# sohamazing/image-stitcher

Measured on AMD Instinct MI355X. Metric: stitched Mvoxels/s, higher is better.
Workload: dtype u16

## Files before the change

### image-stitcher_amd/csrc/fuse.hip

```cpp
#include <hip/hip_runtime.h>

#include <algorithm>
#include <cstdlib>
#include <map>

#include "common.h"

using namespace sq;

namespace {

typedef uint32_t u32x4 __attribute__((ext_vector_type(4)));
typedef float f32x4 __attribute__((ext_vector_type(4)));
typedef double f64x2 __attribute__((ext_vector_type(2)));

struct __attribute__((packed)) U32x4U {
    u32x4 v;
};
struct __attribute__((packed)) F32x4U {
    f32x4 v;
};
typedef uint32_t u32x2 __attribute__((ext_vector_type(2)));
struct __attribute__((packed)) U32x2U {
    u32x2 v;
// ... 1697 lines not shown
        }
    }
}

template <typename K>
int launch(K kernel, const FuseParams &P, int64_t n_items, int n_planes, hipStream_t stream, int grid_override = 0) {
    const int64_t n_work = n_items * n_planes;
    if (n_work == 0) return SQ_OK;
    static thread_local std::map<const void *, int> resident;
    const void *key = reinterpret_cast<const void *>(kernel);
    auto it = resident.find(key);
    if (it == resident.end()) {
        int dev = 0, cus = 256, per_cu = 8;
        hipDeviceProp_t prop;
        if (hipGetDevice(&dev) == hipSuccess && hipGetDeviceProperties(&prop, dev) == hipSuccess)
            cus = prop.multiProcessorCount;
        if (hipOccupancyMaxActiveBlocksPerMultiprocessor(&per_cu, kernel, 256, 0) != hipSuccess || per_cu < 1) per_cu = 4;
        it = resident.emplace(key, cus * std::min(per_cu, 8)).first;
    }
    const int64_t blocks = std::min<int64_t>(n_work, grid_override > 0 ? grid_override : it->second);
    FuseParams Q = P;
    Q.chunk = (int32_t)std::max<int64_t>(1, std::min<int64_t>(QUEUE_CHUNK, n_work / (blocks * 16)));
    hipLaunchKernelGGL(kernel, dim3((unsigned)blocks), dim3(256), 0, stream, Q, n_items, n_work);
    hipError_t e = hipGetLastError();
    if (e != hipSuccess) return fail(SQ_ERR_HIP, "sq_fuse_planes: launch failed: %s", hipGetErrorString(e));
    return SQ_OK;
}

template <typename K>
int launch_zg(K kernel, const FuseParams &P, int64_t n_items, int n_planes, hipStream_t stream, int grid_override) {
    if (n_items == 0 || n_planes == 0) return SQ_OK;
    static thread_local std::map<const void *, int> resident;
    const void *key = reinterpret_cast<const void *>(kernel);
    auto it = resident.find(key);
    if (it == resident.end()) {
        int dev = 0, cus = 256, per_cu = 8;
        hipDeviceProp_t prop;
        if (hipGetDevice(&dev) == hipSuccess && hipGetDeviceProperties(&prop, dev) == hipSuccess)
            cus = prop.multiProcessorCount;
        if (hipOccupancyMaxActiveBlocksPerMultiprocessor(&per_cu, kernel, 256, 0) != hipSuccess || per_cu < 1) per_cu = 4;
        it = resident.emplace(key, cus * std::min(per_cu, 8)).first;
    }
    const int64_t min_units = n_items * ((n_planes + ZB - 1) / ZB);
    const int64_t blocks = std::min<int64_t>(min_units, grid_override > 0 ? grid_override : it->second);
    FuseParams Q = P;
    Q.chunk = (int32_t)std::max<int64_t>(1, std::min<int64_t>(QUEUE_CHUNK, min_units / (blocks * 16)));
    hipLaunchKernelGGL(kernel, dim3((unsigned)blocks), dim3(256), 0, stream, Q, n_items);
    hipError_t e = hipGetLastError();
    if (e != hipSuccess) return fail(SQ_ERR_HIP, "sq_fuse_planes: launch failed: %s", hipGetErrorString(e));
    return SQ_OK;
}

template <typename G>
__global__ __launch_bounds__(256) void flat_classify_kernel(const void *const *flat_ptrs, int64_t n, uint32_t *cls) {
    const int plane = blockIdx.y;
    const G *f = static_cast<const G *>(flat_ptrs[plane]);
    if (!f) return;
    for (int q = 0; q < plane; ++q)
        if (flat_ptrs[q] == f) return;
    const G lo = (G)__builtin_ldexp(1.0, FAST_MIN_EXP), hi = (G)__builtin_ldexp(1.0, FAST_END_EXP);
    const G mlo = (G)__builtin_ldexp(1.0, -MODERATE_EXP), mhi = (G)__builtin_ldexp(1.0, MODERATE_EXP);
    bool odd = false, wide = false, neg = false;
    auto look = [&](G g) {
        const G a = g < 0 ? -g : g;
        odd |= !(a >= lo && a < hi);
        wide |= !(a >= mlo && a < mhi);
        neg |= !(g > 0);
    };
    constexpr int PER = 16 / sizeof(G);
    const int64_t head = min<int64_t>(n, (int64_t)((16 - (reinterpret_cast<uintptr_t>(f) & 15)) & 15) / (int64_t)sizeof(G));
    const int64_t nvec = (n - head) / PER;
    const int64_t tid = (int64_t)blockIdx.x * blockDim.x + threadIdx.x, nthr = (int64_t)gridDim.x * blockDim.x;
    for (int64_t v = tid; v < nvec; v += nthr) {
        if constexpr (sizeof(G) == 4) {
            const f32x4 q = *reinterpret_cast<const f32x4 *>(f + head + v * PER);
            look(q[0]), look(q[1]), look(q[2]), look(q[3]);
        } else {
            const F64x2U q = *reinterpret_cast<const F64x2U *>(f + head + v * PER);
            look(q.v[0]), look(q.v[1]);
        }
    }
    for (int64_t i = tid; i < head; i += nthr) look(ldg_s<G>(f + i));
    for (int64_t i = head + nvec * PER + tid; i < n; i += nthr) look(ldg_s<G>(f + i));
    const uint32_t bits = (__builtin_amdgcn_ballot_w64(odd) ? 1u : 0u) | (__builtin_amdgcn_ballot_w64(wide) ? 2u : 0u) |
                          (__builtin_amdgcn_ballot_w64(neg) ? 4u : 0u);
    if (bits && (threadIdx.x & 63) == 0) atomicOr(&cls[plane], bits);
}

__global__ __launch_bounds__(256) void flat_class_share_kernel(const void *const *flat_ptrs, int n_planes, uint32_t *cls) {
    for (int p = threadIdx.x; p < n_planes; p += 256) {
        const void *f = flat_ptrs[p];
        if (!f) continue;
        for (int q = 0; q < p; ++q)
            if (flat_ptrs[q] == f) {
                cls[p] = cls[q];
                break;
            }
    }
}

__global__ __launch_bounds__(256) void selftest_divide_kernel(int exponent0, int negative, unsigned long long *bad) {
    const uint32_t mant = blockIdx.x * 256u + threadIdx.x;
    const int exponent = exponent0 + (int)blockIdx.y;
    const uint32_t bits = ((uint32_t)(exponent + 127) << 23) | mant | (negative ? 0x80000000u : 0u);
    const float g = __uint_as_float(bits);
    unsigned long long local = 0;
    for (int v = 0; v < 65536; ++v)
    {
        const uint32_t want = flat_f32<uint16_t>((uint16_t)v, g);
        const uint32_t pair = flat_f32_fast_pair((uint32_t)v | ((uint32_t)v << 16), g, g);
        local += want != flat_f32_fast<uint16_t>((uint16_t)v, g);
        local += want != (pair & 0xFFFFu);
        local += want != (pair >> 16);
        local += flat_f32<uint16_t, 1>((uint16_t)v, g) != flat_f32_fast<uint16_t, 1>((uint16_t)v, g);
        local += __fdiv_rn((float)v, g) != div_u16_normal_ieee((float)v, g);
    }
    for (int off = 32; off > 0; off >>= 1) local += __shfl_xor(local, off);
    if ((threadIdx.x & 63) == 0 && local) atomicAdd(bad, local);
}

}

extern "C" int sq_selftest_flat_divide(int32_t exponent, int32_t n_binades, int32_t negative, uint64_t *mismatches_dev,
                                       void *stream) {
    if (!mismatches_dev || exponent < FAST_MIN_EXP || n_binades < 1 || exponent + n_binades > FAST_END_EXP)
        return fail(SQ_ERR_INVALID, "sq_selftest_flat_divide: binades [%d, %d] outside the fast path's range [%d, %d]",
                    exponent, exponent + n_binades - 1, FAST_MIN_EXP, FAST_END_EXP - 1);
    hipStream_t s = static_cast<hipStream_t>(stream);
    hipError_t e = hipMemsetAsync(mismatches_dev, 0, sizeof(uint64_t), s);
    if (e == hipSuccess) {
        hipLaunchKernelGGL(selftest_divide_kernel, dim3(1u << 15, n_binades), dim3(256), 0, s, exponent, negative,
                           reinterpret_cast<unsigned long long *>(mismatches_dev));
        e = hipGetLastError();
    }
    if (e != hipSuccess) return fail(SQ_ERR_HIP, "sq_selftest_flat_divide: %s", hipGetErrorString(e));
    return SQ_OK;
}

__global__ __launch_bounds__(256) void selftest_blend_divide_kernel(int exponent0, int negative, unsigned long long *bad) {
    const uint32_t mant = blockIdx.x * 256u + threadIdx.x;
    const int exponent = exponent0 + (int)blockIdx.y;
    const float acc = __uint_as_float(((uint32_t)(exponent + 127) << 23) | mant | (negative ? 0x80000000u : 0u));
    unsigned long long local = 0;
    for (int ws = 2; ws <= BLEND_WSUM_MAX; ++ws) {
        const float d = (float)ws;
        const float want = __fdiv_rn(acc, d), got = div_by_refined(acc, d, recip_for<1>(d));
        local += __float_as_uint(want) != __float_as_uint(got);
    }
    if (local) atomicAdd(bad, local);
}

// ... 42 lines not shown
    if (!mismatches_dev || exponent < FAST_MIN_EXP || n_binades < 1 || exponent + n_binades > FAST_END_EXP)
        return fail(SQ_ERR_INVALID, "sq_selftest_flat_divide_f64: binades [%d, %d] outside the fast path's range [%d, %d]",
                    exponent, exponent + n_binades - 1, FAST_MIN_EXP, FAST_END_EXP - 1);
    hipStream_t s = static_cast<hipStream_t>(stream);
    hipError_t e = hipMemsetAsync(mismatches_dev, 0, sizeof(uint64_t), s);
    if (e == hipSuccess) {
        hipLaunchKernelGGL(selftest_divide_f64_kernel, dim3(128, n_binades), dim3(256), 0, s, exponent, negative, seed,
                           reinterpret_cast<unsigned long long *>(mismatches_dev));
        e = hipGetLastError();
    }
    if (e != hipSuccess) return fail(SQ_ERR_HIP, "sq_selftest_flat_divide_f64: %s", hipGetErrorString(e));
    return SQ_OK;
}

namespace {
struct ScratchLayout {
    int64_t queue, n_groups, groups, total;
};
ScratchLayout scratch_layout(int64_t n_planes) {
    ScratchLayout L;
    L.queue = (n_planes * 4 + 127) & ~int64_t(127);
    L.n_groups = L.queue + 9 * QUEUE_STRIDE * 4;
    L.groups = L.n_groups + 128;
    L.total = L.groups + n_planes * (int64_t)sizeof(PlaneGroup);
    return L;
}
}

extern "C" int64_t sq_fuse_scratch_bytes(int32_t n_planes) {
    if (n_planes < 0) return fail(SQ_ERR_INVALID, "sq_fuse_scratch_bytes: n_planes %d", n_planes);
    return scratch_layout(n_planes).total;
}

extern "C" int sq_fuse_planes(const sq_fuse_args *a, void *stream_) {
    if (!a || !a->plan || !a->table_dev || !a->canvas_dev)
        return fail(SQ_ERR_INVALID, "sq_fuse_planes: NULL plan/table/canvas");
    const TableHeader &h = a->plan->header();
    if (a->plan->spans_only && !a->plan->expanded)
        return fail(SQ_ERR_INVALID, "sq_fuse_planes: the plan of sq_fuse_plan_create_spans has not been through sq_fuse_plan_expand");
    if (a->table_bytes != a->plan->device_bytes())
        return fail(SQ_ERR_INVALID, "sq_fuse_planes: table_bytes %lld != plan %lld", (long long)a->table_bytes,
                    (long long)a->plan->device_bytes());
    if (a->mode != h.mode) return fail(SQ_ERR_INVALID, "sq_fuse_planes: mode %d but plan was built for %d", a->mode, h.mode);
    if (a->n_tiles != h.n_tiles || a->tile_h != h.tile_h || a->tile_w != h.tile_w || a->canvas_h != h.canvas_h ||
        a->canvas_w != h.canvas_w)
        return fail(SQ_ERR_INVALID, "sq_fuse_planes: geometry differs from the plan (tiles %d/%d %dx%d/%dx%d canvas %dx%d/%dx%d)",
                    a->n_tiles, h.n_tiles, a->tile_h, a->tile_w, h.tile_h, h.tile_w, a->canvas_h, a->canvas_w, h.canvas_h,
                    h.canvas_w);
    if (!a->tile_ptrs_dev && !a->tile_base_dev && h.n_refs > 0)
        return fail(SQ_ERR_INVALID, "sq_fuse_planes: no tile table and no tile base");
    if (a->tile_pitch < a->tile_w || a->canvas_pitch < a->canvas_w)
        return fail(SQ_ERR_INVALID, "sq_fuse_planes: pitch smaller than width");
    if (a->n_planes < 0) return fail(SQ_ERR_INVALID, "sq_fuse_planes: n_planes %d out of range", a->n_planes);
    if ((a->flags & ~(SQ_FUSE_FORCE_QUEUES | SQ_FUSE_FORCE_STATIC | SQ_FUSE_NO_PLANE_GROUPS | SQ_FUSE_NO_SEAM_OWNERS | SQ_FUSE_CONSECUTIVE_GROUPS)) || a->grid_blocks < 0 ||
        ((a->flags & SQ_FUSE_FORCE_QUEUES) && (a->flags & SQ_FUSE_FORCE_STATIC)))
        return fail(SQ_ERR_INVALID, "sq_fuse_planes: flags %d / grid_blocks %d", a->flags, a->grid_blocks);
    if (a->tile_dtype != SQ_U8 && a->tile_dtype != SQ_U16)
        return fail(SQ_ERR_UNSUPPORTED, "sq_fuse_planes: tile dtype %d (uint8/uint16 only)", a->tile_dtype);
    if (a->flat_ptrs_dev && a->flat_dtype != SQ_F32 && a->flat_dtype != SQ_F64)
        return fail(SQ_ERR_UNSUPPORTED, "sq_fuse_planes: flatfield dtype %d (float32/float64 only)", a->flat_dtype);
    if (a->canvas_plane_stride < (int64_t)a->canvas_h * a->canvas_pitch && a->n_planes > 1)
        return fail(SQ_ERR_INVALID, "sq_fuse_planes: canvas planes overlap");
    const size_t esz = a->canvas_dtype == SQ_F32 ? 4 : (size_t)a->canvas_dtype;
    if (reinterpret_cast<uintptr_t>(a->canvas_dev) % esz)
        return fail(SQ_ERR_INVALID, "sq_fuse_planes: canvas pointer not aligned to its element size");

    FuseParams P{};
    const char *base = static_cast<const char *>(a->table_dev);
    P.spans = reinterpret_cast<const Span *>(base + h.off_spans);
    P.refs = reinterpret_cast<const Ref *>(base + h.off_refs);
    P.items = reinterpret_cast<const Item *>(base + h.off_items);
    P.seams = (h.off_seams && !(a->flags & SQ_FUSE_NO_SEAM_OWNERS)) ? reinterpret_cast<const Seam *>(base + h.off_seams) : nullptr;
    P.tile_ptrs = a->tile_ptrs_dev;
    P.tile_base = a->tile_base_dev;
    P.tile_plane_stride = a->tile_plane_stride;
    P.tile_stride = a->tile_stride;
    P.flat_ptrs = a->flat_ptrs_dev;
    P.canvas = a->canvas_dev;
    P.canvas_plane_stride = a->canvas_plane_stride;
    P.n_tiles = a->n_tiles;
    P.tile_h = a->tile_h;
    P.tile_w = a->tile_w;
    P.tile_pitch = a->tile_pitch;
    P.canvas_pitch = a->canvas_pitch;
    P.flat_class = nullptr;
    hipStream_t stream = static_cast<hipStream_t>(stream_);
    const int flat = a->flat_ptrs_dev ? (a->flat_dtype == SQ_F64 ? 2 : 1) : 0;
    P.queue = nullptr;
    P.lane_items = (int32_t)h.lane_items;
    P.n_planes = a->n_planes;
    const ScratchLayout SL = scratch_layout(a->n_planes);
    if (a->scratch_dev && a->n_planes > 0) {
        if (a->scratch_bytes < sq_fuse_scratch_bytes(a->n_planes))
            return fail(SQ_ERR_WORKSPACE, "sq_fuse_planes: scratch %lld < %lld bytes", (long long)a->scratch_bytes,
                        (long long)sq_fuse_scratch_bytes(a->n_planes));
        if (reinterpret_cast<uintptr_t>(a->scratch_dev) % 128) return fail(SQ_ERR_INVALID, "sq_fuse_planes: scratch not 128-byte aligned");
        if (hipMemsetAsync(a->scratch_dev, 0, (size_t)SL.groups, stream) != hipSuccess)
            return fail(SQ_ERR_HIP, "sq_fuse_planes: cannot clear the scratch");
        if (flat) {
            if (flat == 1)
                hipLaunchKernelGGL(flat_classify_kernel<float>, dim3(256, a->n_planes), dim3(256), 0, stream, a->flat_ptrs_dev,
                                   (int64_t)a->tile_h * a->tile_w, static_cast<uint32_t *>(a->scratch_dev));
            else
                hipLaunchKernelGGL(flat_classify_kernel<double>, dim3(256, a->n_planes), dim3(256), 0, stream, a->flat_ptrs_dev,
                                   (int64_t)a->tile_h * a->tile_w, static_cast<uint32_t *>(a->scratch_dev));
            if (a->n_planes > 1)
                hipLaunchKernelGGL(flat_class_share_kernel, dim3(1), dim3(256), 0, stream, a->flat_ptrs_dev, a->n_planes,
                                   static_cast<uint32_t *>(a->scratch_dev));
            P.flat_class = static_cast<const uint32_t *>(a->scratch_dev);
        }
        const int64_t n_work = (int64_t)a->n_planes * h.n_items;
        if ((n_work >= 100000 || (a->flags & SQ_FUSE_FORCE_QUEUES)) && n_work < (int64_t(1) << 31) && !(a->flags & SQ_FUSE_FORCE_STATIC))
            P.queue = reinterpret_cast<uint32_t *>(static_cast<char *>(a->scratch_dev) + SL.queue);
    }
    const bool u16 = a->tile_dtype == SQ_U16;
    const bool grouping = a->scratch_dev && a->n_planes > 1 && ZB > 1 && !(a->flags & SQ_FUSE_NO_PLANE_GROUPS);
    auto build_groups = [&](const void *const *gains, uint32_t cls_mask) {
        char *sc = static_cast<char *>(a->scratch_dev);
        uint32_t *n_groups = reinterpret_cast<uint32_t *>(sc + SL.n_groups);
        PlaneGroup *groups = reinterpret_cast<PlaneGroup *>(sc + SL.groups);
        hipLaunchKernelGGL(build_groups_kernel, dim3(1), dim3(256), 0, stream, gains, P.flat_class, cls_mask, a->n_planes,
                           a->canvas_plane_stride * (int64_t)esz, ZB, n_groups, groups,
                           (a->flags & SQ_FUSE_CONSECUTIVE_GROUPS) != 0);
        P.groups = groups;
        P.n_groups = n_groups;
    };

    if (a->mode == SQ_FUSE_OVERWRITE) {
        if (a->canvas_dtype != a->tile_dtype)
            return fail(SQ_ERR_INVALID, "sq_fuse_planes: overwrite mode keeps the tile dtype (canvas %d, tile %d)",
                        a->canvas_dtype, a->tile_dtype);
#define SQ_OVERWRITE(T, F)                                                                                  \
    do {                                                                                                      \
        if (P.queue) return launch(fuse_overwrite_kernel<T, F, true>, P, h.n_items, a->n_planes, stream, a->grid_blocks);     \
        return launch(fuse_overwrite_kernel<T, F, false>, P, h.n_items, a->n_planes, stream, a->grid_blocks);                 \
    } while (0)
        if (flat && grouping) {
            build_groups(a->flat_ptrs_dev, 1u);
#define SQ_ZG(G, T)                                                                                                                  \
    do {                                                                                                                              \
        if (P.queue) return launch_zg(fuse_overwrite_zg_kernel<G, true, T>, P, h.n_items, a->n_planes, stream, a->grid_blocks);       \
        return launch_zg(fuse_overwrite_zg_kernel<G, false, T>, P, h.n_items, a->n_planes, stream, a->grid_blocks);                   \
    } while (0)
            if (u16) {
                if (flat == 2) SQ_ZG(double, uint16_t);
                SQ_ZG(float, uint16_t);
            }
            if (flat == 2) SQ_ZG(double, uint8_t);
            SQ_ZG(float, uint8_t);
        }
        if (u16 && !flat && grouping) {
            build_groups(nullptr, 0u);
            SQ_ZG(NoGain, uint16_t);
#undef SQ_ZG
        }
        if (u16) {
            if (flat == 0) SQ_OVERWRITE(uint16_t, 0);
            if (flat == 1) SQ_OVERWRITE(uint16_t, 1);
            SQ_OVERWRITE(uint16_t, 2);
        }
        if (flat == 0) SQ_OVERWRITE(uint8_t, 0);
        if (flat == 1) SQ_OVERWRITE(uint8_t, 1);
        SQ_OVERWRITE(uint8_t, 2);
#undef SQ_OVERWRITE
    }
    const bool f32out = a->canvas_dtype == SQ_F32;
    if (!f32out && a->canvas_dtype != a->tile_dtype)
        return fail(SQ_ERR_INVALID, "sq_fuse_planes: feather canvas must be float32 or the tile dtype");
#define SQ_FEATHER_F(T, O, F)                                                                              \
    do {                                                                                                    \
        if (P.queue) return launch(fuse_feather_kernel<T, O, F, true>, P, h.n_items, a->n_planes, stream, a->grid_blocks);  \
        return launch(fuse_feather_kernel<T, O, F, false>, P, h.n_items, a->n_planes, stream, a->grid_blocks);              \
    } while (0)
#define SQ_FEATHER(T, O)                 \
    do {                                 \
        if (flat == 0) SQ_FEATHER_F(T, O, 0); \
// ... 187 lines not shown
        for (int64_t w = blockIdx.x; w < n_work; w += gridDim.x) body(sgpr(P.items[w]));
        return;
    }
    for_each_queued_item<ProjAux>(
        P, n_items, 1u, [&](int, const Item &, int64_t) -> ProjAux { return ProjAux{0}; },
        [&](int, const Item &it, const ProjAux &) { body(it); });
}


template <typename K, typename... X>
int launch_project(const char *who, K kernel, const FuseParams &P, int64_t n_items, hipStream_t stream, int grid_override,
                   X... extra) {
    if (n_items == 0) return SQ_OK;
    static thread_local std::map<const void *, int> resident;
    const void *key = reinterpret_cast<const void *>(kernel);
    auto it = resident.find(key);
    if (it == resident.end()) {
        int dev = 0, cus = 256, per_cu = 8;
        hipDeviceProp_t prop;
        if (hipGetDevice(&dev) == hipSuccess && hipGetDeviceProperties(&prop, dev) == hipSuccess)
            cus = prop.multiProcessorCount;
        if (hipOccupancyMaxActiveBlocksPerMultiprocessor(&per_cu, kernel, 256, 0) != hipSuccess || per_cu < 1) per_cu = 4;
        it = resident.emplace(key, cus * std::min(per_cu, 8)).first;
    }
    const int64_t blocks = std::min<int64_t>(n_items, grid_override > 0 ? grid_override : it->second);
    FuseParams Q = P;
    Q.chunk = (int32_t)std::max<int64_t>(1, std::min<int64_t>(QUEUE_CHUNK, n_items / (blocks * 16)));
    hipLaunchKernelGGL(kernel, dim3((unsigned)blocks), dim3(256), 0, stream, Q, n_items, n_items, extra...);
    hipError_t e = hipGetLastError();
    if (e != hipSuccess) return fail(SQ_ERR_HIP, "%s: launch failed: %s", who, hipGetErrorString(e));
    return SQ_OK;
}

int project_setup(const char *who, const sq_fuse_args *a, int32_t flags, hipStream_t stream, FuseParams &P, int32_t *fl_out) {
    if (!a || !a->plan || !a->table_dev || !a->canvas_dev) return fail(SQ_ERR_INVALID, "%s: NULL plan/table/output", who);
    if (a->mode != SQ_FUSE_OVERWRITE)
        return fail(SQ_ERR_INVALID, "%s: mode %d, only SQ_FUSE_OVERWRITE plans can be projected", who, a->mode);
    const TableHeader &h = a->plan->header();
    if (h.mode != SQ_FUSE_OVERWRITE) return fail(SQ_ERR_INVALID, "%s: the plan was built for mode %d", who, h.mode);
    if (a->plan->spans_only && !a->plan->expanded)
        return fail(SQ_ERR_INVALID, "%s: the plan of sq_fuse_plan_create_spans has not been through sq_fuse_plan_expand", who);
    if (a->table_bytes != a->plan->device_bytes())
        return fail(SQ_ERR_INVALID, "%s: table_bytes %lld != plan %lld", who, (long long)a->table_bytes,
                    (long long)a->plan->device_bytes());
    if (a->n_tiles != h.n_tiles || a->tile_h != h.tile_h || a->tile_w != h.tile_w || a->canvas_h != h.canvas_h ||
        a->canvas_w != h.canvas_w)
        return fail(SQ_ERR_INVALID, "%s: geometry differs from the plan", who);
    if (!a->tile_ptrs_dev && !a->tile_base_dev && h.n_refs > 0)
        return fail(SQ_ERR_INVALID, "%s: no tile table and no tile base", who);
    if (a->tile_pitch < a->tile_w || a->canvas_pitch < a->canvas_w) return fail(SQ_ERR_INVALID, "%s: pitch smaller than width", who);
    if (a->n_planes < 1) return fail(SQ_ERR_INVALID, "%s: n_planes %d (at least one plane)", who, a->n_planes);
    const int32_t fl = flags | a->flags;
    if ((fl & ~(SQ_FUSE_FORCE_QUEUES | SQ_FUSE_FORCE_STATIC | SQ_FUSE_NO_PLANE_GROUPS | SQ_FUSE_NO_SEAM_OWNERS | SQ_FUSE_CONSECUTIVE_GROUPS |
                SQ_PROJECT_ACCUMULATE)) ||
        a->grid_blocks < 0 || ((fl & SQ_FUSE_FORCE_QUEUES) && (fl & SQ_FUSE_FORCE_STATIC)))
        return fail(SQ_ERR_INVALID, "%s: flags %d / grid_blocks %d", who, fl, a->grid_blocks);
    if (a->tile_dtype != SQ_U8 && a->tile_dtype != SQ_U16)
        return fail(SQ_ERR_UNSUPPORTED, "%s: tile dtype %d (uint8/uint16 only)", who, a->tile_dtype);
    if (a->canvas_dtype != a->tile_dtype)
        return fail(SQ_ERR_INVALID, "%s: the output keeps the tile dtype (output %d, tile %d)", who, a->canvas_dtype, a->tile_dtype);
    if (a->flat_ptrs_dev && a->flat_dtype != SQ_F32 && a->flat_dtype != SQ_F64)
        return fail(SQ_ERR_UNSUPPORTED, "%s: flatfield dtype %d (float32/float64 only)", who, a->flat_dtype);
    if (reinterpret_cast<uintptr_t>(a->canvas_dev) % (size_t)a->canvas_dtype)
        return fail(SQ_ERR_INVALID, "%s: output pointer not aligned to its element size", who);

    P = FuseParams{};
    const char *base = static_cast<const char *>(a->table_dev);
    P.spans = reinterpret_cast<const Span *>(base + h.off_spans);
    P.refs = reinterpret_cast<const Ref *>(base + h.off_refs);
    P.items = reinterpret_cast<const Item *>(base + h.off_items);
    P.seams = nullptr;
    P.tile_ptrs = a->tile_ptrs_dev;
    P.tile_base = a->tile_base_dev;
    P.tile_plane_stride = a->tile_plane_stride;
    P.tile_stride = a->tile_stride;
    P.flat_ptrs = a->flat_ptrs_dev;
    P.canvas = a->canvas_dev;
    P.canvas_plane_stride = 0;
    P.n_tiles = a->n_tiles;
    P.tile_h = a->tile_h;
    P.tile_w = a->tile_w;
    P.tile_pitch = a->tile_pitch;
    P.canvas_pitch = a->canvas_pitch;
    P.lane_items = (int32_t)h.lane_items;
    P.n_planes = a->n_planes;
    if (a->scratch_dev) {
        const ScratchLayout SL = scratch_layout(a->n_planes);
        if (a->scratch_bytes < SL.total)
            return fail(SQ_ERR_WORKSPACE, "%s: scratch %lld < %lld bytes", who, (long long)a->scratch_bytes, (long long)SL.total);
        if (reinterpret_cast<uintptr_t>(a->scratch_dev) % 128) return fail(SQ_ERR_INVALID, "%s: scratch not 128-byte aligned", who);
        const int64_t n_work = (int64_t)a->n_planes * h.n_items;
        if ((n_work >= 100000 || (fl & SQ_FUSE_FORCE_QUEUES)) && h.n_items < (int64_t(1) << 31) && !(fl & SQ_FUSE_FORCE_STATIC)) {
            if (hipMemsetAsync(static_cast<char *>(a->scratch_dev) + SL.queue, 0, 9 * QUEUE_STRIDE * 4, stream) != hipSuccess)
                return fail(SQ_ERR_HIP, "%s: cannot clear the queue counters", who);
            P.queue = reinterpret_cast<uint32_t *>(static_cast<char *>(a->scratch_dev) + SL.queue);
        }
    } else if (fl & SQ_FUSE_FORCE_QUEUES) {
        return fail(SQ_ERR_INVALID, "%s: SQ_FUSE_FORCE_QUEUES needs scratch_dev", who);
    }
    *fl_out = fl;
    return SQ_OK;
}
}

extern "C" int sq_fuse_project_max(const sq_fuse_args *a, int32_t flags, void *stream_) {
    static const char *who = "sq_fuse_project_max";
    hipStream_t stream = static_cast<hipStream_t>(stream_);
// ... 541 lines not shown
```

### image-stitcher_amd/native.py

```python
from __future__ import annotations

import ctypes as C
import os
from typing import Optional, Sequence

import numpy as np

_HERE = os.path.dirname(os.path.abspath(__file__))
LIB_PATH = os.environ.get('SQ_LIB_PATH') or os.path.join(_HERE, 'csrc', 'libsquidstitch.so')

SQ_U8, SQ_U16, SQ_F32, SQ_F64 = 1, 2, 4, 8
SQ_FUSE_OVERWRITE, SQ_FUSE_FEATHER = 0, 1
SQ_NORM_NONE, SQ_NORM_PHASE = 0, 1
SQ_FUSE_FORCE_QUEUES, SQ_FUSE_FORCE_STATIC, SQ_FUSE_NO_PLANE_GROUPS, SQ_FUSE_NO_SEAM_OWNERS, SQ_FUSE_CONSECUTIVE_GROUPS = 1, 2, 4, 8, 16
SQ_PROJECT_ACCUMULATE = 32
SQ_FOCUS_ACCUMULATE = 32
SQ_SELECT_ACCUMULATE = 32
SQ_FOCUS_MAX_RADIUS = 15
SQ_FOCUS_MAX_PLANES = 256
SQ_VERSION = 108
SQ_ARENA_NATURAL_ORDER = 1
SQ_ARENA_TWO_CLASSES = 2
SQ_ARENA_MAX_CLASSES = 8

RECT_DTYPE = np.dtype([('src_y0', '<i4'), ('src_x0', '<i4'), ('h', '<i4'), ('w', '<i4'),
                       ('dst_y', '<i4'), ('dst_x', '<i4')])
PAIR_DTYPE = np.dtype([('ref_tile', '<i4'), ('mov_tile', '<i4'), ('ref_y0', '<i4'), ('ref_x0', '<i4'),
                       ('mov_y0', '<i4'), ('mov_x0', '<i4')])
RESULT_DTYPE = np.dtype([('coarse', '<i4', (2,)), ('fine', '<i4', (2,)), ('ccmax_re', '<f8'),
                         ('ccmax_im', '<f8'), ('src_amp', '<f8'), ('tgt_amp', '<f8')])
SYNTH_DTYPE = np.dtype([('scene_seed', '<u8'), ('noise_seed', '<u8'), ('oy', '<i8'), ('ox', '<i8')])
OVERLAP_BATCH = 65535
OVERLAP_DTYPE = np.dtype([('ref_tile', '<i4'), ('mov_tile', '<i4'), ('ref_y0', '<i4'), ('ref_x0', '<i4'),
                          ('mov_y0', '<i4'), ('mov_x0', '<i4'), ('h', '<i4'), ('w', '<i4')])


class NativeError(RuntimeError):
    """A libsquidstitch call returned a negative status."""


class _FuseArgs(C.Structure):
    _fields_ = [
        ('plan', C.c_void_p), ('table_dev', C.c_void_p), ('table_bytes', C.c_int64),
        ('tile_ptrs_dev', C.c_void_p), ('tile_base_dev', C.c_void_p),
        ('tile_plane_stride', C.c_int64), ('tile_stride', C.c_int64),
        ('n_tiles', C.c_int32), ('tile_h', C.c_int32), ('tile_w', C.c_int32),
        ('tile_pitch', C.c_int32), ('tile_dtype', C.c_int32),
        ('flat_ptrs_dev', C.c_void_p), ('flat_dtype', C.c_int32),
        ('canvas_dev', C.c_void_p), ('canvas_plane_stride', C.c_int64),
        ('canvas_h', C.c_int32), ('canvas_w', C.c_int32), ('canvas_pitch', C.c_int32),
        ('canvas_dtype', C.c_int32), ('n_planes', C.c_int32), ('mode', C.c_int32),
        ('scratch_dev', C.c_void_p), ('scratch_bytes', C.c_int64),
        ('flags', C.c_int32), ('grid_blocks', C.c_int32),
    ]


class _FocusArgs(C.Structure):
    _fields_ = [
        ('z_levels_dev', C.c_void_p), ('radius', C.c_int32),
        ('scratch_dev', C.c_void_p), ('scratch_bytes', C.c_int64),
        ('key_dev', C.c_void_p), ('key_pitch', C.c_int32),
    ]


class _RegisterArgs(C.Structure):
    _fields_ = [
        ('tile_ptrs_dev', C.c_void_p), ('tile_base_dev', C.c_void_p), ('tile_stride', C.c_int64),
# ... 260 lines not shown
    if tile_ptrs is not None:
        if tile_ptrs.dtype != torch.int64 or tile_ptrs.numel() != n_planes * plan.n_tiles:
            raise ValueError("tile_ptrs must be int64 with n_planes * n_tiles entries")
        a.tile_ptrs_dev = tile_ptrs.data_ptr()
        a.tile_base_dev = None
        tile_np = np_dtype_of_torch(out.dtype) if plan.mode == SQ_FUSE_OVERWRITE else np.dtype('uint16')
        if tiles is not None:
            tile_np = np_dtype_of_torch(tiles.dtype)
    else:
        if tiles is None or not tiles.is_cuda or not tiles.is_contiguous():
            raise ValueError("tiles must be a contiguous device tensor")
        if tiles.numel() != n_planes * plan.n_tiles * plan.tile_h * plan.tile_w:
            raise ValueError(f"tiles has {tiles.numel()} elements, expected "
                             f"{n_planes}x{plan.n_tiles}x{plan.tile_h}x{plan.tile_w}")
        a.tile_ptrs_dev = None
        a.tile_base_dev = tiles.data_ptr()
        a.tile_stride = plan.tile_h * plan.tile_w
        a.tile_plane_stride = plan.n_tiles * plan.tile_h * plan.tile_w
        tile_np = np_dtype_of_torch(tiles.dtype)
    a.n_tiles, a.tile_h, a.tile_w, a.tile_pitch = plan.n_tiles, plan.tile_h, plan.tile_w, plan.tile_w
    a.tile_dtype = sq_dtype_of(tile_np)
    a.flat_ptrs_dev = None
    a.flat_dtype = SQ_F32
    if flats is not None and any(f is not None for f in flats):
        if len(flats) != n_planes:
            raise ValueError("flats needs one entry per plane")
        dts = {f.dtype for f in flats if f is not None}
        if len(dts) != 1:
            raise ValueError("all flatfields must share one dtype")
        for f in flats:
            if f is not None and (tuple(f.shape) != (plan.tile_h, plan.tile_w) or not f.is_contiguous()):
                raise ValueError("flatfield must be a contiguous tile_h x tile_w tensor")
        a.flat_dtype = sq_dtype_of(np_dtype_of_torch(dts.pop()))
        fp = flat_ptrs if flat_ptrs is not None else pointer_table(flats, out.device)
        if fp.dtype != torch.int64 or fp.numel() != n_planes:
            raise ValueError("flat_ptrs must be int64 with one entry per plane")
        keep.append(fp)
        a.flat_ptrs_dev = fp.data_ptr()
    if n_planes > 0:
        scratch = torch.empty(int(L.sq_fuse_scratch_bytes(n_planes)), dtype=torch.uint8, device=out.device)
        keep.append(scratch)
        a.scratch_dev = scratch.data_ptr()
        a.scratch_bytes = scratch.numel()
    a.canvas_dev = out.data_ptr()
    a.canvas_plane_stride = plane_stride
    a.canvas_h, a.canvas_w, a.canvas_pitch = hc, wc, pitch
    a.canvas_dtype = sq_dtype_of(np_dtype_of_torch(out.dtype))
    a.n_planes = n_planes
    a.mode = plan.mode
    return a


def fuse_planes(plan: FusePlan, tiles, canvas, flats=None, tile_ptrs=None, stream=None, flat_ptrs=None,
                flags: int = 0, grid_blocks: int = 0) -> None:
    L = lib()
    hc, wc = int(canvas.shape[-2]), int(canvas.shape[-1])
    n_planes = int(canvas.numel() // (hc * wc)) if hc * wc else 0
    pitch, plane_stride = wc, hc * wc
    if not canvas.is_cuda:
        raise ValueError("canvas must be a device tensor")
    if not canvas.is_contiguous():
        if canvas.dim() != 3 or (wc > 1 and canvas.stride(2) != 1) or canvas.stride(1) < wc or \
                (n_planes > 1 and canvas.stride(0) < (hc - 1) * canvas.stride(1) + wc):
            raise ValueError("canvas must be contiguous or a [P, Hc, Wc] tensor with unit-stride rows and non-overlapping planes")
        pitch, plane_stride = int(canvas.stride(1)), int(canvas.stride(0))
    keep = []
    a = _fuse_args(plan, tiles, n_planes, canvas, plane_stride, pitch, flats, tile_ptrs, flat_ptrs, keep)
    a.flags, a.grid_blocks = int(flags), int(grid_blocks)
    if stream is not None:
        for t in keep:
            t.record_stream(stream)
    _check(L.sq_fuse_planes(C.byref(a), _stream_ptr(stream)), 'sq_fuse_planes')


def fuse_project_max(plan: FusePlan, tiles, out, flats=None, tile_ptrs=None, accumulate: bool = False, flags: int = 0,
                     stream=None, flat_ptrs=None, grid_blocks: int = 0) -> None:
    L = lib()
    if plan.mode != SQ_FUSE_OVERWRITE:
        raise ValueError("fuse_project_max projects overwrite plans only")
    if not out.is_cuda or out.dim() != 2 or tuple(out.shape) != (plan.canvas_h, plan.canvas_w):
        raise ValueError(f"out must be a [{plan.canvas_h}, {plan.canvas_w}] device tensor")
    hc, wc = int(out.shape[0]), int(out.shape[1])
    if (wc > 1 and out.stride(1) != 1) or (hc > 1 and out.stride(0) < wc):
        raise ValueError("out must have unit-stride rows")
    pitch = int(out.stride(0)) if hc > 1 else wc
    if tile_ptrs is not None:
        n_planes = int(tile_ptrs.numel()) // max(plan.n_tiles, 1) if plan.n_tiles else (len(flats) if flats is not None else 1)
    elif tiles is not None:
        n_planes = int(tiles.shape[0]) if tiles.dim() == 4 else 1
    else:
        raise ValueError("tiles or tile_ptrs is required")
    if n_planes < 1:
        raise ValueError("at least one plane to project")
    keep = []
    a = _fuse_args(plan, tiles, n_planes, out, 0, pitch, flats, tile_ptrs, flat_ptrs, keep)
    a.flags, a.grid_blocks = 0, int(grid_blocks)
    if stream is not None:
        for t in keep:
            t.record_stream(stream)
    fl = int(flags) | (SQ_PROJECT_ACCUMULATE if accumulate else 0)
    _check(L.sq_fuse_project_max(C.byref(a), fl, _stream_ptr(stream)), 'sq_fuse_project_max')


def focus_scratch_bytes(n_tiles: int, tile_h: int, tile_w: int) -> int:
    n = int(lib().sq_focus_scratch_bytes(int(n_tiles), int(tile_h), int(tile_w)))
    if n < 0:
        _check(n, 'sq_focus_scratch_bytes')
    return n


def fuse_project_focus(plan: FusePlan, tiles, out, key, z_levels, radius: int = 3, flats=None, scratch=None,
                       accumulate: bool = False, tile_ptrs=None, flags: int = 0, stream=None, flat_ptrs=None,
                       grid_blocks: int = 0) -> None:
    import torch
    L = lib()
    if plan.mode != SQ_FUSE_OVERWRITE:
        raise ValueError("fuse_project_focus projects overwrite plans only")
    if not 0 <= int(radius) <= SQ_FOCUS_MAX_RADIUS:
        raise ValueError(f"focus radius {radius} outside 0..{SQ_FOCUS_MAX_RADIUS}")
    shape = (plan.canvas_h, plan.canvas_w)
    for name, t in (('out', out), ('key', key)):
        if not t.is_cuda or t.dim() != 2 or tuple(t.shape) != shape:
            raise ValueError(f"{name} must be a [{shape[0]}, {shape[1]}] device tensor")
        if (shape[1] > 1 and t.stride(1) != 1) or (shape[0] > 1 and t.stride(0) < shape[1]):
            raise ValueError(f"{name} must have unit-stride rows")
# ... 605 lines not shown
```

### include/squidstitch.h

```cpp
#ifndef SQUIDSTITCH_H
#define SQUIDSTITCH_H

#include <stddef.h>
#include <stdint.h>

#ifdef __cplusplus
extern "C" {
#endif

#define SQ_VERSION 108

typedef enum sq_status {
    SQ_OK = 0,
    SQ_ERR_INVALID = -1,
    SQ_ERR_HIP = -2,
    SQ_ERR_UNSUPPORTED = -3,
    SQ_ERR_WORKSPACE = -4
} sq_status;

typedef enum sq_dtype { SQ_U8 = 1, SQ_U16 = 2, SQ_F32 = 4, SQ_F64 = 8 } sq_dtype;

int sq_version(void);
const char *sq_last_error(void);

// ... 5 lines not shown
} sq_rect;

typedef enum sq_fuse_mode {
    SQ_FUSE_OVERWRITE = 0,
    SQ_FUSE_FEATHER = 1
} sq_fuse_mode;

typedef struct sq_fuse_plan sq_fuse_plan;

sq_fuse_plan *sq_fuse_plan_create(const sq_rect *rects, int32_t n_rects, int32_t tile_h, int32_t tile_w,
                                  int32_t canvas_h, int32_t canvas_w, int32_t mode);
void sq_fuse_plan_destroy(sq_fuse_plan *plan);
int64_t sq_fuse_plan_table_bytes(const sq_fuse_plan *plan);
int sq_fuse_plan_export(const sq_fuse_plan *plan, void *host_buf, int64_t host_bytes);

int sq_fuse_plan_upload(const sq_fuse_plan *plan, void *table_dev, int64_t table_bytes, void *stream);
sq_fuse_plan *sq_fuse_plan_create_spans(const sq_rect *rects, int32_t n_rects, int32_t tile_h, int32_t tile_w,
                                        int32_t canvas_h, int32_t canvas_w, int32_t mode);
int64_t sq_fuse_plan_expand_scratch_bytes(const sq_fuse_plan *plan);
int sq_fuse_plan_expand(sq_fuse_plan *plan, void *table_dev, int64_t table_bytes, void *scratch_dev, int64_t scratch_bytes,
                        void *stream);
int sq_fuse_plan_stats(const sq_fuse_plan *plan, int64_t *n_spans, int64_t *n_items, int64_t *covered_voxels,
                       int32_t *max_refs);

typedef struct sq_fuse_args {
    const sq_fuse_plan *plan;
    const void *table_dev;
    int64_t table_bytes;
    const void *const *tile_ptrs_dev;
    const void *tile_base_dev;
    int64_t tile_plane_stride, tile_stride;
    int32_t n_tiles, tile_h, tile_w;
    int32_t tile_pitch;
    int32_t tile_dtype;
    const void *const *flat_ptrs_dev;
    int32_t flat_dtype;
    void *canvas_dev;
    int64_t canvas_plane_stride;
    int32_t canvas_h, canvas_w, canvas_pitch;
    int32_t canvas_dtype;
    int32_t n_planes;
    int32_t mode;
    void *scratch_dev;
    int64_t scratch_bytes;
    int32_t flags;
    int32_t grid_blocks;
} sq_fuse_args;

typedef enum sq_fuse_flags {
    SQ_FUSE_FORCE_QUEUES = 1,
    SQ_FUSE_FORCE_STATIC = 2,
    SQ_FUSE_NO_PLANE_GROUPS = 4,
    SQ_FUSE_NO_SEAM_OWNERS = 8,
    SQ_FUSE_CONSECUTIVE_GROUPS = 16
} sq_fuse_flags;

int64_t sq_fuse_scratch_bytes(int32_t n_planes);

int sq_fuse_planes(const sq_fuse_args *args, void *stream);

#define SQ_PROJECT_ACCUMULATE 32
int sq_fuse_project_max(const sq_fuse_args *args, int32_t flags, void *stream);

#define SQ_FOCUS_ACCUMULATE 32
#define SQ_FOCUS_MAX_RADIUS 15
#define SQ_FOCUS_MAX_PLANES 256
typedef struct sq_focus_args {
    const uint32_t *z_levels_dev;
    int32_t radius;
    void *scratch_dev;
    int64_t scratch_bytes;
    void *key_dev;
    int32_t key_pitch;
} sq_focus_args;
int64_t sq_focus_scratch_bytes(int32_t n_tiles, int32_t tile_h, int32_t tile_w);
int sq_fuse_project_focus(const sq_fuse_args *args, const sq_focus_args *focus, int32_t flags, void *stream);

#define SQ_SELECT_ACCUMULATE 32
int sq_focus_depth_plane(const void *key_dev, int32_t key_pitch, int32_t h, int32_t w, void *depth_dev, int32_t depth_pitch,
                         int32_t depth_dtype, void *stream);
int sq_fuse_select_depth(const sq_fuse_args *args, const void *depth_dev, int32_t depth_pitch, int32_t depth_dtype,
                         const uint32_t *z_levels_dev, int32_t flags, void *stream);

#define SQ_ARENA_MAX_CLASSES 8
typedef enum sq_arena_flags { SQ_ARENA_NATURAL_ORDER = 1, SQ_ARENA_TWO_CLASSES = 2 } sq_arena_flags;
typedef struct sq_arena sq_arena;
typedef struct sq_arena_info {
    void *base_dev;
    int64_t bytes;
    int64_t slice_bytes;
    int32_t n_slices;
    int32_t n_candidates;
    int32_t n_classes;
    int32_t class_slices[SQ_ARENA_MAX_CLASSES];
    int32_t class_candidates[SQ_ARENA_MAX_CLASSES];
    int32_t interleaved;
    float probe_ms;
    float create_ms;
    float min_pair_gbs, max_pair_gbs;
} sq_arena_info;
sq_arena *sq_arena_create(int64_t bytes, int64_t candidate_bytes, int64_t slice_bytes, int64_t unit_bytes, int32_t flags,
                          void *stream, sq_arena_info *info);
int sq_arena_info_get(const sq_arena *arena, sq_arena_info *info);
int sq_arena_destroy(sq_arena *arena);

int sq_downsample2(const void *src_dev, int64_t src_plane_stride, int32_t src_h, int32_t src_w, int64_t src_pitch,
                   void *dst_dev, int64_t dst_plane_stride, int64_t dst_pitch, int32_t n_planes, int32_t dtype,
// ... 110 lines not shown
```

Before: 1.592 million.

## Fuse flat-field classification, class sharing and plane grouping into one prepass kernel

Replaces the separate classify, class-share and build-groups kernel launches with a single prepass kernel. The last-arriving block, detected through an atomic counter, propagates classes to duplicate planes and builds the plane groups in shared memory. The aim is to cut launch overhead and serialised tiny kernels ahead of the main fuse kernel. It adds a last-block pattern that relies on threadfences, and it is capped at 256 planes, with a flag to fall back to the split path.

```diff
diff --git a/image-stitcher_amd/csrc/fuse.hip b/image-stitcher_amd/csrc/fuse.hip
--- a/image-stitcher_amd/csrc/fuse.hip
+++ b/image-stitcher_amd/csrc/fuse.hip
@@ -1773,12 +1773,7 @@
 }
 
 template <typename G>
-__global__ __launch_bounds__(256) void flat_classify_kernel(const void *const *flat_ptrs, int64_t n, uint32_t *cls) {
-    const int plane = blockIdx.y;
-    const G *f = static_cast<const G *>(flat_ptrs[plane]);
-    if (!f) return;
-    for (int q = 0; q < plane; ++q)
-        if (flat_ptrs[q] == f) return;
+__device__ __forceinline__ uint32_t flat_class_bits(const G *f, int64_t n, int64_t tid, int64_t nthr) {
     const G lo = (G)__builtin_ldexp(1.0, FAST_MIN_EXP), hi = (G)__builtin_ldexp(1.0, FAST_END_EXP);
     const G mlo = (G)__builtin_ldexp(1.0, -MODERATE_EXP), mhi = (G)__builtin_ldexp(1.0, MODERATE_EXP);
     bool odd = false, wide = false, neg = false;
@@ -1791,7 +1786,6 @@
     constexpr int PER = 16 / sizeof(G);
     const int64_t head = min<int64_t>(n, (int64_t)((16 - (reinterpret_cast<uintptr_t>(f) & 15)) & 15) / (int64_t)sizeof(G));
     const int64_t nvec = (n - head) / PER;
-    const int64_t tid = (int64_t)blockIdx.x * blockDim.x + threadIdx.x, nthr = (int64_t)gridDim.x * blockDim.x;
     for (int64_t v = tid; v < nvec; v += nthr) {
         if constexpr (sizeof(G) == 4) {
             const f32x4 q = *reinterpret_cast<const f32x4 *>(f + head + v * PER);
@@ -1803,8 +1797,18 @@
     }
     for (int64_t i = tid; i < head; i += nthr) look(ldg_s<G>(f + i));
     for (int64_t i = head + nvec * PER + tid; i < n; i += nthr) look(ldg_s<G>(f + i));
-    const uint32_t bits = (__builtin_amdgcn_ballot_w64(odd) ? 1u : 0u) | (__builtin_amdgcn_ballot_w64(wide) ? 2u : 0u) |
-                          (__builtin_amdgcn_ballot_w64(neg) ? 4u : 0u);
+    return (__builtin_amdgcn_ballot_w64(odd) ? 1u : 0u) | (__builtin_amdgcn_ballot_w64(wide) ? 2u : 0u) |
+           (__builtin_amdgcn_ballot_w64(neg) ? 4u : 0u);
+}
+
+template <typename G>
+__global__ __launch_bounds__(256) void flat_classify_kernel(const void *const *flat_ptrs, int64_t n, uint32_t *cls) {
+    const int plane = blockIdx.y;
+    const G *f = static_cast<const G *>(flat_ptrs[plane]);
+    if (!f) return;
+    for (int q = 0; q < plane; ++q)
+        if (flat_ptrs[q] == f) return;
+    const uint32_t bits = flat_class_bits<G>(f, n, (int64_t)blockIdx.x * blockDim.x + threadIdx.x, (int64_t)gridDim.x * blockDim.x);
     if (bits && (threadIdx.x & 63) == 0) atomicOr(&cls[plane], bits);
 }
 
@@ -1818,6 +1822,80 @@
                 break;
             }
     }
+}
+
+constexpr int PREPASS_CAP = 256;
+template <typename G>
+__global__ __launch_bounds__(256) void fuse_prepass_kernel(const void *const *flat_ptrs, int64_t n, uint32_t *cls, int n_planes,
+                                                          uint32_t *arrived, bool want_groups, uint32_t cls_mask,
+                                                          int64_t plane_stride_bytes, int zb, uint32_t *n_groups,
+                                                          PlaneGroup *groups, bool consecutive) {
+    __shared__ uint64_t s_key[PREPASS_CAP];
+    __shared__ int s_slots[PREPASS_CAP], s_open[PREPASS_CAP], s_group[PREPASS_CAP];
+    __shared__ PlaneGroup s_out[PREPASS_CAP];
+    __shared__ uint8_t s_distinct[PREPASS_CAP];
+    __shared__ int s_last;
+    const int tid = threadIdx.x;
+    const bool mine = tid < n_planes;
+    const void *const f_mine = mine ? flat_ptrs[tid] : nullptr;
+    int lead = tid;
+    if (f_mine)
+        for (int q = tid - 1; q >= 0; --q)
+            if (flat_ptrs[q] == f_mine) lead = q;
+    if (mine) s_distinct[tid] = f_mine && lead == tid;
+    __syncthreads();
+    const int64_t gtid = (int64_t)blockIdx.x * blockDim.x + tid, nthr = (int64_t)gridDim.x * blockDim.x;
+    for (int p = 0; p < n_planes; ++p) {
+        if (!s_distinct[p]) continue;
+        const uint32_t bits = flat_class_bits<G>(static_cast<const G *>(flat_ptrs[p]), n, gtid, nthr);
+        if (bits && (tid & 63) == 0) atomicOr(&cls[p], bits);
+    }
+    __threadfence();
+    __syncthreads();
+    if (tid == 0) {
+        __threadfence();
+        s_last = atomicAdd(arrived, 1u) == gridDim.x - 1;
+    }
+    __syncthreads();
+    if (!s_last) return;
+    __threadfence();
+    const uint32_t c = f_mine ? __hip_atomic_load(&cls[lead], __ATOMIC_RELAXED, __HIP_MEMORY_SCOPE_AGENT) : 0u;
+    if (f_mine && lead != tid) cls[tid] = c;
+    if (!want_groups) return;
+    const bool ok = f_mine && (c & cls_mask) == 0;
+    const uint64_t key =
+        ok ? ((reinterpret_cast<uint64_t>(f_mine) << 7) | (uint64_t)(((int64_t)tid * plane_stride_bytes) & 127) | (1ull << 63)) : 0;
+    if (mine) s_key[tid] = key;
+    __syncthreads();
+    int j = 0, m = 0, klead = tid;
+    if (mine && key)
+        for (int q = n_planes - 1; q >= 0; --q) {
+            const bool eq = s_key[q] == key;
+            m += eq;
+            if (q < tid && eq) ++j, klead = q;
+        }
+    const int key_groups = (m + zb - 1) / zb;
+    if (mine) s_slots[tid] = !key ? 1 : (klead == tid ? key_groups : 0);
+    __syncthreads();
+    int open = 0, ng = 0;
+    for (int q = 0; q < n_planes; ++q) {
+        const int k = s_slots[q];
+        ng += k;
+        if (q < tid) open += k;
+    }
+    if (mine) s_open[tid] = open;
+    __syncthreads();
+    if (mine) s_group[tid] = key ? s_open[klead] + (consecutive ? j / zb : j % key_groups) : open;
+    __syncthreads();
+    if (tid < ng) {
+        int cnt = 0;
+        for (int q = 0; q < n_planes; ++q)
+            if (s_group[q] == tid && cnt < 7) s_out[tid].plane[cnt++] = q;
+        s_out[tid].n = cnt;
+        for (int z = cnt; z < 7; ++z) s_out[tid].plane[z] = s_out[tid].plane[0];
+        groups[tid] = s_out[tid];
+    }
+    if (tid == 0) *n_groups = (uint32_t)ng;
 }
 
 __global__ __launch_bounds__(256) void selftest_divide_kernel(int exponent0, int negative, unsigned long long *bad) {
@@ -1966,7 +2044,8 @@
     if (a->tile_pitch < a->tile_w || a->canvas_pitch < a->canvas_w)
         return fail(SQ_ERR_INVALID, "sq_fuse_planes: pitch smaller than width");
     if (a->n_planes < 0) return fail(SQ_ERR_INVALID, "sq_fuse_planes: n_planes %d out of range", a->n_planes);
-    if ((a->flags & ~(SQ_FUSE_FORCE_QUEUES | SQ_FUSE_FORCE_STATIC | SQ_FUSE_NO_PLANE_GROUPS | SQ_FUSE_NO_SEAM_OWNERS | SQ_FUSE_CONSECUTIVE_GROUPS)) || a->grid_blocks < 0 ||
+    if ((a->flags & ~(SQ_FUSE_FORCE_QUEUES | SQ_FUSE_FORCE_STATIC | SQ_FUSE_NO_PLANE_GROUPS | SQ_FUSE_NO_SEAM_OWNERS | SQ_FUSE_CONSECUTIVE_GROUPS |
+                      SQ_FUSE_SPLIT_PREPASS)) || a->grid_blocks < 0 ||
         ((a->flags & SQ_FUSE_FORCE_QUEUES) && (a->flags & SQ_FUSE_FORCE_STATIC)))
         return fail(SQ_ERR_INVALID, "sq_fuse_planes: flags %d / grid_blocks %d", a->flags, a->grid_blocks);
     if (a->tile_dtype != SQ_U8 && a->tile_dtype != SQ_U16)
@@ -2004,6 +2083,10 @@
     P.lane_items = (int32_t)h.lane_items;
     P.n_planes = a->n_planes;
     const ScratchLayout SL = scratch_layout(a->n_planes);
+    const bool u16 = a->tile_dtype == SQ_U16;
+    const bool grouping = a->scratch_dev && a->n_planes > 1 && ZB > 1 && !(a->flags & SQ_FUSE_NO_PLANE_GROUPS);
+    bool fused_groups = false;
+    uint32_t fused_mask = 0;
     if (a->scratch_dev && a->n_planes > 0) {
         if (a->scratch_bytes < sq_fuse_scratch_bytes(a->n_planes))
             return fail(SQ_ERR_WORKSPACE, "sq_fuse_planes: scratch %lld < %lld bytes", (long long)a->scratch_bytes,
@@ -2011,7 +2094,30 @@
         if (reinterpret_cast<uintptr_t>(a->scratch_dev) % 128) return fail(SQ_ERR_INVALID, "sq_fuse_planes: scratch not 128-byte aligned");
         if (hipMemsetAsync(a->scratch_dev, 0, (size_t)SL.groups, stream) != hipSuccess)
             return fail(SQ_ERR_HIP, "sq_fuse_planes: cannot clear the scratch");
-        if (flat) {
+        if (flat && a->n_planes <= PREPASS_CAP && !(a->flags & SQ_FUSE_SPLIT_PREPASS)) {
+            if (grouping && a->mode == SQ_FUSE_OVERWRITE) {
+                fused_groups = true;
+                fused_mask = 1u;
+            } else if (grouping && a->mode != SQ_FUSE_OVERWRITE && u16 && std::min(a->tile_h, a->tile_w) <= BLEND_WSUM_MAX) {
+                fused_groups = true;
+                fused_mask = a->canvas_dtype == SQ_F32 ? 7u : 3u;
+            }
+            char *sc = static_cast<char *>(a->scratch_dev);
+            uint32_t *cls = static_cast<uint32_t *>(a->scratch_dev);
+            uint32_t *n_groups = reinterpret_cast<uint32_t *>(sc + SL.n_groups);
+            uint32_t *arrived = n_groups + 16;
+            PlaneGroup *groups = reinterpret_cast<PlaneGroup *>(sc + SL.groups);
+            const dim3 grid(256u * (unsigned)std::min(a->n_planes, 8));
+            const int64_t n_gain = (int64_t)a->tile_h * a->tile_w, stride_bytes = a->canvas_plane_stride * (int64_t)esz;
+            const bool consecutive = (a->flags & SQ_FUSE_CONSECUTIVE_GROUPS) != 0;
+            if (flat == 1)
+                hipLaunchKernelGGL(fuse_prepass_kernel<float>, grid, dim3(256), 0, stream, a->flat_ptrs_dev, n_gain, cls,
+                                   a->n_planes, arrived, fused_groups, fused_mask, stride_bytes, ZB, n_groups, groups, consecutive);
+            else
+                hipLaunchKernelGGL(fuse_prepass_kernel<double>, grid, dim3(256), 0, stream, a->flat_ptrs_dev, n_gain, cls,
+                                   a->n_planes, arrived, fused_groups, fused_mask, stride_bytes, ZB, n_groups, groups, consecutive);
+            P.flat_class = cls;
+        } else if (flat) {
             if (flat == 1)
                 hipLaunchKernelGGL(flat_classify_kernel<float>, dim3(256, a->n_planes), dim3(256), 0, stream, a->flat_ptrs_dev,
                                    (int64_t)a->tile_h * a->tile_w, static_cast<uint32_t *>(a->scratch_dev));
@@ -2027,15 +2133,15 @@
         if ((n_work >= 100000 || (a->flags & SQ_FUSE_FORCE_QUEUES)) && n_work < (int64_t(1) << 31) && !(a->flags & SQ_FUSE_FORCE_STATIC))
             P.queue = reinterpret_cast<uint32_t *>(static_cast<char *>(a->scratch_dev) + SL.queue);
     }
-    const bool u16 = a->tile_dtype == SQ_U16;
-    const bool grouping = a->scratch_dev && a->n_planes > 1 && ZB > 1 && !(a->flags & SQ_FUSE_NO_PLANE_GROUPS);
     auto build_groups = [&](const void *const *gains, uint32_t cls_mask) {
         char *sc = static_cast<char *>(a->scratch_dev);
         uint32_t *n_groups = reinterpret_cast<uint32_t *>(sc + SL.n_groups);
         PlaneGroup *groups = reinterpret_cast<PlaneGroup *>(sc + SL.groups);
-        hipLaunchKernelGGL(build_groups_kernel, dim3(1), dim3(256), 0, stream, gains, P.flat_class, cls_mask, a->n_planes,
-                           a->canvas_plane_stride * (int64_t)esz, ZB, n_groups, groups,
-                           (a->flags & SQ_FUSE_CONSECUTIVE_GROUPS) != 0);
+        if (!(fused_groups && gains && cls_mask == fused_mask)) {
+            hipLaunchKernelGGL(build_groups_kernel, dim3(1), dim3(256), 0, stream, gains, P.flat_class, cls_mask, a->n_planes,
+                               a->canvas_plane_stride * (int64_t)esz, ZB, n_groups, groups,
+                               (a->flags & SQ_FUSE_CONSECUTIVE_GROUPS) != 0);
+        }
         P.groups = groups;
         P.n_groups = n_groups;
     };
@@ -2329,7 +2435,7 @@
     if (a->n_planes < 1) return fail(SQ_ERR_INVALID, "%s: n_planes %d (at least one plane)", who, a->n_planes);
     const int32_t fl = flags | a->flags;
     if ((fl & ~(SQ_FUSE_FORCE_QUEUES | SQ_FUSE_FORCE_STATIC | SQ_FUSE_NO_PLANE_GROUPS | SQ_FUSE_NO_SEAM_OWNERS | SQ_FUSE_CONSECUTIVE_GROUPS |
-                SQ_PROJECT_ACCUMULATE)) ||
+                SQ_FUSE_SPLIT_PREPASS | SQ_PROJECT_ACCUMULATE)) ||
         a->grid_blocks < 0 || ((fl & SQ_FUSE_FORCE_QUEUES) && (fl & SQ_FUSE_FORCE_STATIC)))
         return fail(SQ_ERR_INVALID, "%s: flags %d / grid_blocks %d", who, fl, a->grid_blocks);
     if (a->tile_dtype != SQ_U8 && a->tile_dtype != SQ_U16)
diff --git a/image-stitcher_amd/native.py b/image-stitcher_amd/native.py
--- a/image-stitcher_amd/native.py
+++ b/image-stitcher_amd/native.py
@@ -13,6 +13,7 @@
 SQ_FUSE_OVERWRITE, SQ_FUSE_FEATHER = 0, 1
 SQ_NORM_NONE, SQ_NORM_PHASE = 0, 1
 SQ_FUSE_FORCE_QUEUES, SQ_FUSE_FORCE_STATIC, SQ_FUSE_NO_PLANE_GROUPS, SQ_FUSE_NO_SEAM_OWNERS, SQ_FUSE_CONSECUTIVE_GROUPS = 1, 2, 4, 8, 16
+SQ_FUSE_SPLIT_PREPASS = 64
 SQ_PROJECT_ACCUMULATE = 32
 SQ_FOCUS_ACCUMULATE = 32
 SQ_SELECT_ACCUMULATE = 32
@@ -379,7 +380,8 @@
 
 
 def fuse_planes(plan: FusePlan, tiles, canvas, flats=None, tile_ptrs=None, stream=None, flat_ptrs=None,
-                flags: int = 0, grid_blocks: int = 0) -> None:
+                flags: int = 0, grid_blocks: int = 0, scratch=None) -> None:
+    import torch
     L = lib()
     hc, wc = int(canvas.shape[-2]), int(canvas.shape[-1])
     n_planes = int(canvas.numel() // (hc * wc)) if hc * wc else 0
@@ -394,10 +396,35 @@
     keep = []
     a = _fuse_args(plan, tiles, n_planes, canvas, plane_stride, pitch, flats, tile_ptrs, flat_ptrs, keep)
     a.flags, a.grid_blocks = int(flags), int(grid_blocks)
+    if scratch is not None and n_planes > 0:
+        if not scratch.is_cuda or scratch.dtype != torch.uint8 or scratch.numel() < fuse_scratch_bytes(n_planes):
+            raise ValueError(f"scratch must be a device uint8 tensor of at least {fuse_scratch_bytes(n_planes)} bytes")
+        keep.append(scratch)
+        a.scratch_dev, a.scratch_bytes = scratch.data_ptr(), scratch.numel()
     if stream is not None:
         for t in keep:
             t.record_stream(stream)
     _check(L.sq_fuse_planes(C.byref(a), _stream_ptr(stream)), 'sq_fuse_planes')
+
+
+def fuse_scratch_bytes(n_planes: int) -> int:
+    n = int(lib().sq_fuse_scratch_bytes(int(n_planes)))
+    if n < 0:
+        _check(n, 'sq_fuse_scratch_bytes')
+    return n
+
+
+def fuse_scratch_view(scratch, n_planes: int):
+    raw = scratch.cpu().numpy().view(np.uint8)
+    off_queue = (4 * n_planes + 127) & ~127
+    off_count = off_queue + 9 * 128
+    off_groups = off_count + 128
+    classes = raw[:4 * n_planes].view(np.uint32).copy()
+    n_groups = int(raw[off_count:off_count + 4].view(np.uint32)[0])
+    if n_groups > n_planes:
+        raise NativeError(f"fuse scratch: {n_groups} groups for {n_planes} planes")
+    groups = raw[off_groups:off_groups + 32 * n_groups].view(np.int32).reshape(n_groups, 8).copy()
+    return classes, n_groups, groups
 
 
 def fuse_project_max(plan: FusePlan, tiles, out, flats=None, tile_ptrs=None, accumulate: bool = False, flags: int = 0,
diff --git a/include/squidstitch.h b/include/squidstitch.h
--- a/include/squidstitch.h
+++ b/include/squidstitch.h
@@ -81,7 +81,8 @@
     SQ_FUSE_FORCE_STATIC = 2,
     SQ_FUSE_NO_PLANE_GROUPS = 4,
     SQ_FUSE_NO_SEAM_OWNERS = 8,
-    SQ_FUSE_CONSECUTIVE_GROUPS = 16
+    SQ_FUSE_CONSECUTIVE_GROUPS = 16,
+    SQ_FUSE_SPLIT_PREPASS = 64
 } sq_fuse_flags;
 
 int64_t sq_fuse_scratch_bytes(int32_t n_planes);
```

Measured after the change: 1.589 million. About the same (-0.2%).
